# hszhao/semseg

Measured on NVIDIA H100. Metric: PSPNet50 473x473 training images/sec, higher is better.
Workload: dtype bf16

## Files before the change

semseg_b200/csrc/conv_igemm.cu:

```cuda
#include "host_common.h"
#include "ptx.cuh"

namespace sb {

constexpr int kBlockM = 128;
constexpr int kBlockK = 64;
constexpr int kConvThreads = 384;
constexpr int kConsumerThreads = 256;
constexpr int kATileBytes = kBlockM * kBlockK * 2;
constexpr int kStageOutBytes = kBlockM * 64 * 2;
constexpr int kMiscBytes = 2048;

template <int BLOCK_N>
struct ConvCfg {
  static constexpr int kBTileBytes = BLOCK_N * kBlockK * 2;
  static constexpr int kStageBytes = kATileBytes + kBTileBytes;
  static constexpr int kStages = (BLOCK_N == 256) ? 4 : (BLOCK_N == 128 ? 6 : 8);
  static constexpr int kSmemBytes = kStages * kStageBytes + 2 * kStageOutBytes + kMiscBytes + 1024;
};

struct ConvKParams {
  int N, H, W;
  int Cin, Cout;
  int taps;
  int bh, bw, tiles_h, tiles_w;
  int n_tiles, num_m_tiles;
  int k_chunks;
  int dh[SEMSEG_MAX_TAPS], dw[SEMSEG_MAX_TAPS], wtap[SEMSEG_MAX_TAPS], img_add[SEMSEG_MAX_TAPS];
  int img_mul;
  int epi_mode, relu;
  const float* scale;
  const float* shift;
  const __nv_bfloat16* residual;
  const __nv_bfloat16* residual_lo;
  int res_pitch;
  int nseg;
  int k_slices, kb_per_slice;
  long long slice_stride;
  float* out_f32;
  int out_pitch;
  float* stats_partial;
};

template <int BLOCK_N, bool kSplit>
__global__ void __launch_bounds__(kConvThreads, 1)
conv_igemm_kernel(const __grid_constant__ CUtensorMap tmA, const __grid_constant__ CUtensorMap tmB,
                  const __grid_constant__ CUtensorMap tmC, const __grid_constant__ CUtensorMap tmA_lo,
                  const __grid_constant__ CUtensorMap tmB_lo, const __grid_constant__ CUtensorMap tmC_lo,
                  const ConvKParams p) {
  using Cfg = ConvCfg<BLOCK_N>;
  constexpr int kStages = Cfg::kStages;
  constexpr int kStageBytes = Cfg::kStageBytes;
  constexpr int kAcc = BLOCK_N / 2;
  const int num_items = p.num_m_tiles * p.n_tiles * p.k_slices;
  auto decode_item = [&](int item, int& m_tile, int& n_tile, int& k_slice) {
    k_slice = item % p.k_slices;
    item /= p.k_slices;
    n_tile = item % p.n_tiles;
    m_tile = item / p.n_tiles;
  };

  extern __shared__ __align__(1024) uint8_t smem_raw[];
  uint8_t* smem = reinterpret_cast<uint8_t*>((reinterpret_cast<uintptr_t>(smem_raw) + 1023) & ~uintptr_t(1023));
  uint8_t* stage_base = smem;
  uint8_t* out_stage = smem + kStages * kStageBytes;
  uint8_t* misc = out_stage + 2 * kStageOutBytes;
  static_assert(kStages <= 16, "barrier area sized for <= 16 stages");
  uint64_t* full_bar = reinterpret_cast<uint64_t*>(misc);
  uint64_t* empty_bar = full_bar + 16;

  const int warp = threadIdx.x >> 5;
  const int lane = threadIdx.x & 31;
  const int nseg = kSplit ? p.nseg : 1;
  const int total_kblk = p.taps * p.k_chunks;
  auto slice_range = [&](int k_slice, int& kblk0, int& kblk1) {
    kblk0 = k_slice * p.kb_per_slice;
    kblk1 = min(kblk0 + p.kb_per_slice, total_kblk);
  };
  const uint32_t stage_tx = static_cast<uint32_t>(p.bh * p.bw) * 128u + static_cast<uint32_t>(Cfg::kBTileBytes);

  if (warp == 0 && lane == 0) {
    tma_prefetch_desc(&tmA);
    tma_prefetch_desc(&tmB);
    tma_prefetch_desc(&tmC);
    if (kSplit) {
      tma_prefetch_desc(&tmA_lo);
      tma_prefetch_desc(&tmB_lo);
      tma_prefetch_desc(&tmC_lo);
    }
    for (int i = 0; i < kStages; ++i) {
      mbar_init(&full_bar[i], 1);
      mbar_init(&empty_bar[i], kConsumerThreads);
    }
    fence_barrier_init();
  }
  if (p.stats_partial != nullptr) {
    float* row = p.stats_partial + static_cast<size_t>(blockIdx.x) * 4 * 3 * p.Cout;
    for (int i = threadIdx.x; i < 4 * 3 * p.Cout; i += kConvThreads) row[i] = 0.f;
  }
  __syncthreads();

  if (warp < 4) {
    setmaxnreg_dec<40>();
    if (warp == 0 && elect_one()) {
      int it = 0;
      for (int item = blockIdx.x; item < num_items; item += gridDim.x) {
        int m_tile, n_tile, k_slice, kblk0, kblk1;
        decode_item(item, m_tile, n_tile, k_slice);
        slice_range(k_slice, kblk0, kblk1);
        const int tiles_per_img = p.tiles_h * p.tiles_w;
        const int img = m_tile / tiles_per_img;
        const int rem = m_tile - img * tiles_per_img;
        const int h0 = (rem / p.tiles_w) * p.bh;
        const int w0 = (rem % p.tiles_w) * p.bw;
        const int n0 = n_tile * BLOCK_N;
        for (int kb = kblk0 * nseg; kb < kblk1 * nseg; ++kb, ++it) {
          const int s = it % kStages;
          const uint32_t par = (it / kStages) & 1;
          mbar_wait(&empty_bar[s], par ^ 1);
          const int ks = kb / nseg;
          const int seg = kb - ks * nseg;
          const int cb = ks / p.taps;
          const int t = ks - cb * p.taps;
          const CUtensorMap* mA = (kSplit && seg == 1) ? &tmA_lo : &tmA;
          const CUtensorMap* mB = (kSplit && seg == 2) ? &tmB_lo : &tmB;
          uint8_t* a_dst = stage_base + s * kStageBytes;
          uint8_t* b_dst = a_dst + kATileBytes;
          mbar_expect_tx(&full_bar[s], stage_tx);
          tma_load_4d(a_dst, mA, &full_bar[s], cb * kBlockK, w0 + p.dw[t], h0 + p.dh[t],
                      img * p.img_mul + p.img_add[t]);
          tma_load_3d(b_dst, mB, &full_bar[s], cb * kBlockK, n0, p.wtap[t]);
        }
      }
    }
  } else {
    setmaxnreg_inc<232>();
    const int ct = threadIdx.x - 128;
    const int wg = ct >> 7;
    const int wq = (ct >> 5) & 3;
    const int r_base = wg * 64 + wq * 16 + (lane >> 2);
    const int cq = 2 * (lane & 3);
    int it = 0;
    int store_buf = 0;
    float acc[kAcc];
    for (int item = blockIdx.x; item < num_items; item += gridDim.x) {
      int m_tile, n_tile, k_slice, kblk0, kblk1;
      decode_item(item, m_tile, n_tile, k_slice);
      slice_range(k_slice, kblk0, kblk1);
      const int num_kb = (kblk1 - kblk0) * nseg;
      int prev_s = -1;
#pragma unroll
      for (int i = 0; i < kAcc; ++i) acc[i] = 0.f;
      for (int kb = 0; kb < num_kb; ++kb, ++it) {
        const int s = it % kStages;
        const uint32_t par = (it / kStages) & 1;
        mbar_wait(&full_bar[s], par);
        const uint32_t a_addr = smem_u32(stage_base + s * kStageBytes) + static_cast<uint32_t>(wg * 64 * 128);
        const uint32_t b_addr = smem_u32(stage_base + s * kStageBytes + kATileBytes);
        const uint64_t adesc = make_wgmma_desc_sw128(a_addr, 16, 1024);
        const uint64_t bdesc = make_wgmma_desc_sw128(b_addr, 16, 1024);
        wgmma_fence_operand(acc);
        wgmma_fence();
#pragma unroll
        for (int k = 0; k < kBlockK / 16; ++k)
          wgmma_bf16<BLOCK_N, 0, 0>(acc, adesc + static_cast<uint64_t>(k * 2), bdesc + static_cast<uint64_t>(k * 2),
                                    (kb > 0 || k > 0) ? 1u : 0u);
        wgmma_commit();
        wgmma_wait<1>();
        wgmma_fence_operand(acc);
        if (prev_s >= 0) mbar_arrive(&empty_bar[prev_s]);
        prev_s = s;
      }
      wgmma_wait<0>();
      wgmma_fence_operand(acc);
      if (prev_s >= 0) mbar_arrive(&empty_bar[prev_s]);

      const int tiles_per_img = p.tiles_h * p.tiles_w;
      const int img = m_tile / tiles_per_img;
      const int rem = m_tile - img * tiles_per_img;
      const int h0 = (rem / p.tiles_w) * p.bh;
      const int w0 = (rem % p.tiles_w) * p.bw;
      const int n0 = n_tile * BLOCK_N;
      auto row_ok = [&](int r) {
        const int hi = r / p.bw, wi = r - (r / p.bw) * p.bw;
        return (r < p.bh * p.bw) && (h0 + hi < p.H) && (w0 + wi < p.W);
      };
      auto row_pix = [&](int r) {
        const int hi = r / p.bw, wi = r - hi * p.bw;
        return (static_cast<long long>(img) * p.H + (h0 + hi)) * p.W + (w0 + wi);
      };
      bool rv[2];
      long long pix[2];
#pragma unroll
      for (int i = 0; i < 2; ++i) {
        rv[i] = row_ok(r_base + 8 * i);
        pix[i] = row_pix(r_base + 8 * i);
      }
      constexpr int kChunks = BLOCK_N / 64;
#pragma unroll
      for (int ch = 0; ch < kChunks; ++ch) {
        const int c0 = n0 + ch * 64;
        if (c0 >= p.Cout) break;
        float* a = acc + ch * 32;

        if (p.epi_mode == SEMSEG_EPI_F32) {
          const bool bias = p.shift != nullptr && k_slice == 0;
          const bool pairs = (p.out_pitch & 1) == 0;
#pragma unroll
          for (int i = 0; i < 2; ++i) {
            if (!rv[i]) continue;
            float* orow = p.out_f32 + k_slice * p.slice_stride + pix[i] * p.out_pitch;
#pragma unroll
            for (int j = 0; j < 8; ++j) {
              const int c = c0 + 8 * j + cq;
              float v0 = a[4 * j + 2 * i], v1 = a[4 * j + 2 * i + 1];
              if (pairs && c + 1 < p.Cout) {
                if (bias) {
                  v0 += __ldg(p.shift + c);
                  v1 += __ldg(p.shift + c + 1);
                }
                *reinterpret_cast<float2*>(orow + c) = make_float2(v0, v1);
              } else {
                if (c < p.Cout) orow[c] = bias ? v0 + __ldg(p.shift + c) : v0;
                if (c + 1 < p.Cout) orow[c + 1] = bias ? v1 + __ldg(p.shift + c + 1) : v1;
              }
            }
          }
          continue;
        }

        if (p.epi_mode == SEMSEG_EPI_AFFINE) {
          const bool has_res = p.residual != nullptr;
#pragma unroll
          for (int j = 0; j < 8; ++j) {
            const int c = c0 + 8 * j + cq;
            const float sc0 = p.scale ? __ldg(p.scale + c) : 1.f, sc1 = p.scale ? __ldg(p.scale + c + 1) : 1.f;
            const float sh0 = p.shift ? __ldg(p.shift + c) : 0.f, sh1 = p.shift ? __ldg(p.shift + c + 1) : 0.f;
#pragma unroll
            for (int i = 0; i < 2; ++i) {
              float r0 = 0.f, r1 = 0.f;
              if (has_res && rv[i]) {
                const long long ro = pix[i] * p.res_pitch + c;
                float2 f = __bfloat1622float2(*reinterpret_cast<const __nv_bfloat162*>(p.residual + ro));
                if constexpr (kSplit) {
                  const float2 fl = __bfloat1622float2(*reinterpret_cast<const __nv_bfloat162*>(p.residual_lo + ro));
                  f.x += fl.x;
                  f.y += fl.y;
                }
                r0 = f.x;
                r1 = f.y;
              }
              float v0 = fmaf(a[4 * j + 2 * i], sc0, sh0) + r0;
              float v1 = fmaf(a[4 * j + 2 * i + 1], sc1, sh1) + r1;
              if (p.relu) {
                v0 = fmaxf(v0, 0.f);
                v1 = fmaxf(v1, 0.f);
              }
              a[4 * j + 2 * i] = v0;
              a[4 * j + 2 * i + 1] = v1;
            }
          }
        }

        uint8_t* obuf = out_stage + (kSplit ? 0 : store_buf) * kStageOutBytes;
        if (ct == 0) tma_store_wait_read<(kSplit ? 0 : 1)>();
        named_bar_sync(1, kConsumerThreads);
#pragma unroll
        for (int j = 0; j < 8; ++j) {
#pragma unroll
          for (int i = 0; i < 2; ++i) {
            const int r = r_base + 8 * i;
            const float v0 = a[4 * j + 2 * i], v1 = a[4 * j + 2 * i + 1];
            const uint32_t h = pack_bf16x2(v0, v1);
            const int off = r * 128 + ((j ^ (r & 7)) << 4) + cq * 2;
            *reinterpret_cast<uint32_t*>(obuf + off) = h;
            if constexpr (kSplit) {
              const float2 hf = __bfloat1622float2(*reinterpret_cast<const __nv_bfloat162*>(&h));
              *reinterpret_cast<uint32_t*>(obuf + kStageOutBytes + off) = pack_bf16x2(v0 - hf.x, v1 - hf.y);
            }
          }
        }
        fence_proxy_async_smem();
        named_bar_sync(1, kConsumerThreads);
        if (ct == 0) {
          tma_store_4d(&tmC, obuf, c0, w0, h0, img);
          if (kSplit) tma_store_4d(&tmC_lo, obuf + kStageOutBytes, c0, w0, h0, img);
          tma_store_commit();
        }
        if (p.stats_partial != nullptr && p.epi_mode == SEMSEG_EPI_RAW && wg == (ch & 1)) {
          const int g = wq;
          float* st_dst = p.stats_partial + (static_cast<size_t>(blockIdx.x) * 4 + g) * 3 * p.Cout + c0 + 2 * lane;
          float st_old[6];
          st_old[0] = st_dst[0];
          st_old[1] = st_dst[1];
          st_old[2] = st_dst[p.Cout];
          st_old[3] = st_dst[p.Cout + 1];
          st_old[4] = st_dst[2 * p.Cout];
          st_old[5] = st_dst[2 * p.Cout + 1];
          const uint32_t row_msk = __ballot_sync(0xffffffffu, row_ok(g * 32 + lane));
          float s0 = 0.f, s1 = 0.f, q0 = 0.f, q1 = 0.f;
          const uint8_t* base = obuf + (lane & 3) * 4;
          const int chunk16 = lane >> 2;
          auto add_row = [&](int rr, int sw) {
            float2 f = __bfloat1622float2(
                *reinterpret_cast<const __nv_bfloat162*>(base + rr * 128 + ((chunk16 ^ sw) << 4)));
            if constexpr (kSplit) {
              const float2 fl = __bfloat1622float2(*reinterpret_cast<const __nv_bfloat162*>(
                  base + kStageOutBytes + rr * 128 + ((chunk16 ^ sw) << 4)));
              f.x += fl.x;
              f.y += fl.y;
            }
            s0 += f.x;
            s1 += f.y;
            q0 = fmaf(f.x, f.x, q0);
            q1 = fmaf(f.y, f.y, q1);
          };
          if ((row_msk & (row_msk + 1u)) == 0u) {
            const int nr = __popc(row_msk);
            const int nfull = nr >> 3;
            for (int b8 = 0; b8 < nfull; ++b8) {
              const int rr0 = g * 32 + b8 * 8;
#pragma unroll
              for (int k = 0; k < 8; ++k) add_row(rr0 + k, k);
            }
            for (int r = nfull * 8; r < nr; ++r) add_row(g * 32 + r, r & 7);
          } else {
#pragma unroll
            for (int r = 0; r < 32; ++r)
              if ((row_msk >> r) & 1u) add_row(g * 32 + r, r & 7);
          }
          const float nt = static_cast<float>(__popc(row_msk));
          st_dst[0] = st_old[0] + s0;
          st_dst[1] = st_old[1] + s1;
          st_dst[p.Cout] = st_old[2] + q0;
          st_dst[p.Cout + 1] = st_old[3] + q1;
          st_dst[2 * p.Cout] = st_old[4] + nt;
          st_dst[2 * p.Cout + 1] = st_old[5] + nt;
        }
        store_buf ^= 1;
      }
    }
    if (ct == 0) tma_store_wait_all<0>();
  }
}

static int conv_grid(int num_m_tiles, int n_tiles) {
  const int sms = num_sms();
  const long long tiles = static_cast<long long>(num_m_tiles) * n_tiles;
  return static_cast<int>(tiles < sms ? tiles : sms);
}

struct ConvMaps {
  CUtensorMap a, b, c, a_lo, b_lo, c_lo;
};

template <int BLOCK_N>
static int launch_conv(const ConvMaps& tm, const ConvKParams& kp, bool split, int grid, cudaStream_t stream) {
  using Cfg = ConvCfg<BLOCK_N>;
  static std::atomic<bool> attr_set[64];
  int dev = 0;
  SB_CUDA(cudaGetDevice(&dev));
  if (dev < 0 || dev >= 64 || !attr_set[dev].load(std::memory_order_acquire)) {
    SB_CUDA(cudaFuncSetAttribute(conv_igemm_kernel<BLOCK_N, false>, cudaFuncAttributeMaxDynamicSharedMemorySize,
                                 Cfg::kSmemBytes));
    SB_CUDA(cudaFuncSetAttribute(conv_igemm_kernel<BLOCK_N, true>, cudaFuncAttributeMaxDynamicSharedMemorySize,
                                 Cfg::kSmemBytes));
    if (dev >= 0 && dev < 64) attr_set[dev].store(true, std::memory_order_release);
  }
  if (split)
    conv_igemm_kernel<BLOCK_N, true><<<grid, kConvThreads, Cfg::kSmemBytes, stream>>>(tm.a, tm.b, tm.c, tm.a_lo,
                                                                                      tm.b_lo, tm.c_lo, kp);
  else
    conv_igemm_kernel<BLOCK_N, false><<<grid, kConvThreads, Cfg::kSmemBytes, stream>>>(tm.a, tm.b, tm.c, tm.a_lo,
                                                                                       tm.b_lo, tm.c_lo, kp);
  SB_LAUNCHED();
  return SEMSEG_OK;
}

}

static int conv_block_n(int Cout) {
  if (Cout % 256 == 0 || Cout > 128) return 256;
  return Cout > 64 ? 128 : 64;
}

extern "C" int semseg_conv_k_slices(int Cin, int taps, int max_kblocks) {
  if (Cin <= 0 || taps <= 0 || max_kblocks <= 0) return SEMSEG_E_INVALID;
  const int total = taps * sb::cdiv(Cin, sb::kBlockK);
  const int per = sb::cdiv(total, sb::cdiv(total, max_kblocks));
  return sb::cdiv(total, per);
}

extern "C" int semseg_conv_stats_rows(int N, int H, int W, int Cout) {
  if (N <= 0 || H <= 0 || W <= 0 || Cout <= 0) return SEMSEG_E_INVALID;
  int bh, bw;
  sb::choose_box(H, W, sb::kBlockM, &bh, &bw);
  return 4 * sb::conv_grid(N * sb::cdiv(H, bh) * sb::cdiv(W, bw), sb::cdiv(Cout, conv_block_n(Cout)));
}

extern "C" int semseg_conv_fprop(const semseg_conv_desc* d, void* stream_) {
  using namespace sb;
  cudaStream_t stream = static_cast<cudaStream_t>(stream_);
  SB_CHECK_ARG(d != nullptr, "conv: null descriptor");
  SB_CHECK_ARG(d->N > 0 && d->H > 0 && d->W > 0 && d->Cin > 0 && d->Cout > 0, "conv: bad sizes");
  SB_CHECK_ARG(d->taps >= 1 && d->taps <= SEMSEG_MAX_TAPS, "conv: taps=%d out of range", d->taps);
  SB_CHECK_ARG(d->x && d->w, "conv: null x/w");
  SB_CHECK_ARG(d->x_pitch % 8 == 0 && d->x_pitch >= d->Cin, "conv: x_pitch %d must be a multiple of 8 and >= Cin",
               d->x_pitch);
  SB_CHECK_ARG(d->w_cols % 8 == 0 && d->w_cols >= d->Cin, "conv: w_cols %d must be a multiple of 8 and >= Cin",
               d->w_cols);
  SB_CHECK_ARG(d->epi_mode >= 0 && d->epi_mode <= 2, "conv: bad epi_mode");

  ConvKParams kp;
  memset(&kp, 0, sizeof(kp));
  kp.N = d->N; kp.H = d->H; kp.W = d->W; kp.Cin = d->Cin; kp.Cout = d->Cout; kp.taps = d->taps;
  choose_box(d->H, d->W, kBlockM, &kp.bh, &kp.bw);
  kp.tiles_h = cdiv(d->H, kp.bh);
  kp.tiles_w = cdiv(d->W, kp.bw);
  kp.num_m_tiles = d->N * kp.tiles_h * kp.tiles_w;
  kp.k_chunks = cdiv(d->Cin, kBlockK);
  for (int t = 0; t < d->taps; ++t) {
    kp.dh[t] = d->dh[t]; kp.dw[t] = d->dw[t]; kp.wtap[t] = d->wtap[t]; kp.img_add[t] = d->img_add[t];
    SB_CHECK_ARG(d->wtap[t] >= 0 && d->wtap[t] < d->n_wtaps, "conv: wtap[%d]=%d out of range", t, d->wtap[t]);
  }
  kp.img_mul = d->img_mul;
  kp.epi_mode = d->epi_mode; kp.relu = d->relu;
  kp.scale = d->scale; kp.shift = d->shift;
  kp.residual = static_cast<const __nv_bfloat16*>(d->residual); kp.res_pitch = d->res_pitch;
  kp.residual_lo = static_cast<const __nv_bfloat16*>(d->residual_lo);
  const bool split = d->x_lo != nullptr;
  kp.nseg = split ? 3 : 1;
  if (split) {
    SB_CHECK_ARG(d->w_split != 0, "conv: split activations need split weights (w_split)");
    SB_CHECK_ARG(d->epi_mode == SEMSEG_EPI_F32 || d->y_lo != nullptr, "conv: split input needs a split output (y_lo)");
    SB_CHECK_ARG(!d->residual || d->residual_lo, "conv: split input needs a split residual (residual_lo)");
  } else {
    SB_CHECK_ARG(!d->y_lo && !d->residual_lo, "conv: lo planes given without x_lo");
  }
  kp.out_f32 = d->out_f32; kp.out_pitch = d->out_pitch;
  kp.stats_partial = d->stats_partial;

  const int block_n = conv_block_n(d->Cout);
  kp.n_tiles = cdiv(d->Cout, block_n);
  kp.k_slices = 1;
  kp.kb_per_slice = kp.taps * kp.k_chunks;
  kp.slice_stride = 0;
  if (d->k_slices > 1) {
    SB_CHECK_ARG(d->epi_mode == SEMSEG_EPI_F32, "conv: K slicing needs the F32 epilogue (partials are fp32)");
    SB_CHECK_ARG(d->slice_stride >= static_cast<long long>(d->N) * d->H * d->W * d->out_pitch,
                 "conv: slice_stride too small for an [N,H,W,out_pitch] partial");
    kp.kb_per_slice = cdiv(kp.taps * kp.k_chunks, d->k_slices);
    kp.k_slices = cdiv(kp.taps * kp.k_chunks, kp.kb_per_slice);
    SB_CHECK_ARG(kp.k_slices == d->k_slices, "conv: k_slices %d not realisable for %d K blocks (use %d)", d->k_slices,
                 kp.taps * kp.k_chunks, kp.k_slices);
    kp.slice_stride = d->slice_stride;
  }
  const int grid = conv_grid(kp.num_m_tiles, kp.n_tiles * kp.k_slices);

  ConvMaps tm;
  {
    uint64_t dims[4] = {(uint64_t)d->Cin, (uint64_t)d->Win, (uint64_t)d->Hin, (uint64_t)d->Nin};
    uint64_t str[3] = {(uint64_t)d->x_pitch * 2, (uint64_t)d->x_pitch * 2 * d->Win,
                       (uint64_t)d->x_pitch * 2 * d->Win * d->Hin};
    uint32_t box[4] = {(uint32_t)kBlockK, (uint32_t)kp.bw, (uint32_t)kp.bh, 1};
    int r = encode_tmap_bf16(&tm.a, d->x, 4, dims, str, box);
    if (r) return r;
    tm.a_lo = tm.a;
    if (split && (r = encode_tmap_bf16(&tm.a_lo, d->x_lo, 4, dims, str, box))) return r;
  }
  {
    uint64_t dims[3] = {(uint64_t)d->w_cols, (uint64_t)d->w_rows, (uint64_t)d->n_wtaps};
    uint64_t str[2] = {(uint64_t)d->w_cols * 2, (uint64_t)d->w_cols * 2 * d->w_rows};
    uint32_t box[3] = {(uint32_t)kBlockK, (uint32_t)block_n, 1};
    int r = encode_tmap_bf16(&tm.b, d->w, 3, dims, str, box);
    if (r) return r;
    tm.b_lo = tm.b;
    if (split) {
      const __nv_bfloat16* w_lo =
          static_cast<const __nv_bfloat16*>(d->w) + static_cast<size_t>(d->n_wtaps) * d->w_rows * d->w_cols;
      if ((r = encode_tmap_bf16(&tm.b_lo, w_lo, 3, dims, str, box))) return r;
    }
  }
  if (d->epi_mode == SEMSEG_EPI_F32) {
    SB_CHECK_ARG(d->out_f32 != nullptr && d->out_pitch >= d->Cout, "conv: F32 epilogue needs out_f32/out_pitch");
    tm.c = tm.a;
    tm.c_lo = tm.a;
  } else {
    SB_CHECK_ARG(d->y != nullptr, "conv: null y");
    SB_CHECK_ARG(d->Cout % 64 == 0, "conv: bf16 epilogue needs Cout %% 64 == 0 (got %d)", d->Cout);
    SB_CHECK_ARG(d->y_pitch % 8 == 0 && d->y_pitch >= d->Cout, "conv: bad y_pitch %d", d->y_pitch);
    if (d->residual) SB_CHECK_ARG(d->res_pitch % 8 == 0, "conv: res_pitch must be a multiple of 8");
    uint64_t dims[4] = {(uint64_t)d->Cout, (uint64_t)d->W, (uint64_t)d->H, (uint64_t)d->N};
    uint64_t str[3] = {(uint64_t)d->y_pitch * 2, (uint64_t)d->y_pitch * 2 * d->W,
                       (uint64_t)d->y_pitch * 2 * d->W * d->H};
    uint32_t box[4] = {64u, (uint32_t)kp.bw, (uint32_t)kp.bh, 1};
    int r = encode_tmap_bf16(&tm.c, d->y, 4, dims, str, box);
    if (r) return r;
    tm.c_lo = tm.c;
    if (split && (r = encode_tmap_bf16(&tm.c_lo, d->y_lo, 4, dims, str, box))) return r;
  }
  switch (block_n) {
    case 256: return launch_conv<256>(tm, kp, split, grid, stream);
    case 128: return launch_conv<128>(tm, kp, split, grid, stream);
    default: return launch_conv<64>(tm, kp, split, grid, stream);
  }
}
```

semseg_b200/csrc/host_common.cu:

```cuda
#include "host_common.h"

#include <cudaTypedefs.h>
#include <stdarg.h>
#include <string.h>

#include <mutex>

namespace sb {

static thread_local char g_err[512] = "";
std::atomic<long long> g_launches{0};

void set_error(const char* fmt, ...) {
  va_list ap;
  va_start(ap, fmt);
  vsnprintf(g_err, sizeof(g_err), fmt, ap);
  va_end(ap);
}

int num_sms() {
  static int cached[64] = {0};
  int dev = 0;
  if (cudaGetDevice(&dev) != cudaSuccess || dev < 0 || dev >= 64) return 148;
  if (cached[dev] == 0) {
// ... 2 lines not shown
    cached[dev] = n;
  }
  return cached[dev];
}

static PFN_cuTensorMapEncodeTiled_v12000 get_encode() {
  static PFN_cuTensorMapEncodeTiled_v12000 fn = nullptr;
  static std::once_flag once;
  std::call_once(once, [] {
    void* p = nullptr;
    cudaDriverEntryPointQueryResult q;
    if (cudaGetDriverEntryPoint("cuTensorMapEncodeTiled", &p, cudaEnableDefault, &q) == cudaSuccess &&
        q == cudaDriverEntryPointSuccess)
      fn = reinterpret_cast<PFN_cuTensorMapEncodeTiled_v12000>(p);
  });
  return fn;
}

int encode_tmap_bf16(CUtensorMap* out, const void* base, int rank, const uint64_t* dims,
                     const uint64_t* strides_bytes, const uint32_t* box) {
  auto fn = get_encode();
  if (!fn) {
    set_error("cuTensorMapEncodeTiled entry point unavailable (no CUDA driver?)");
    return SEMSEG_E_CUDA;
  }
  if ((reinterpret_cast<uintptr_t>(base) & 15) != 0) {
    set_error("tensor base %p not 16-byte aligned", base);
    return SEMSEG_E_INVALID;
  }
  cuuint64_t gd[5];
  cuuint64_t gs[4];
  cuuint32_t bx[5], es[5];
  for (int i = 0; i < rank; ++i) {
    gd[i] = dims[i];
    bx[i] = box[i];
    es[i] = 1;
    if (box[i] == 0 || box[i] > 256) {
      set_error("TMA box dim %d = %u out of range", i, box[i]);
      return SEMSEG_E_INVALID;
    }
  }
  for (int i = 0; i + 1 < rank; ++i) {
    gs[i] = strides_bytes[i];
    if (gs[i] % 16 != 0) {
      set_error("TMA stride %d = %llu not a multiple of 16 bytes", i, (unsigned long long)gs[i]);
      return SEMSEG_E_INVALID;
    }
  }
  CUresult r = fn(out, CU_TENSOR_MAP_DATA_TYPE_BFLOAT16, rank, const_cast<void*>(base), gd, gs, bx, es,
                  CU_TENSOR_MAP_INTERLEAVE_NONE, CU_TENSOR_MAP_SWIZZLE_128B, CU_TENSOR_MAP_L2_PROMOTION_L2_256B,
                  CU_TENSOR_MAP_FLOAT_OOB_FILL_NONE);
  if (r != CUDA_SUCCESS) {
    set_error("cuTensorMapEncodeTiled failed with CUresult %d (rank %d dims %llu,%llu,%llu box %u,%u,%u)", (int)r,
              rank, (unsigned long long)gd[0], (unsigned long long)gd[1], (unsigned long long)(rank > 2 ? gd[2] : 0),
              bx[0], bx[1], rank > 2 ? bx[2] : 0);
    return SEMSEG_E_CUDA;
  }
  return SEMSEG_OK;
}

void choose_box(int H, int W, int max_pixels, int* bh_out, int* bw_out) {
  double best = -1.0;
  int best_bh = 1, best_bw = 1;
  int wcap = W < max_pixels ? W : max_pixels;
  for (int bw = 1; bw <= wcap; ++bw) {
    int bh = max_pixels / bw;
    if (bh > H) bh = H;
    if (bh > 256) bh = 256;
    if (bh < 1) continue;
    int th = cdiv(H, bh);
    bh = cdiv(H, th);
    int tw = cdiv(W, bw);
    double util = (double)H * W / ((double)th * tw * max_pixels);
    if (util > best + 1e-9 || (util > best - 1e-9 && bw > best_bw)) {
      best = util;
      best_bh = bh;
      best_bw = bw;
    }
  }
  *bh_out = best_bh;
  *bw_out = best_bw;
}

}

extern "C" const char* semseg_last_error(void) { return sb::g_err; }
extern "C" int semseg_abi_version(void) { return 1; }
extern "C" long long semseg_launch_count(void) { return sb::g_launches.load(); }
```

semseg_b200/csrc/host_common.h:

```cpp
#pragma once
#include <cuda.h>
#include <cuda_runtime.h>
#include <stdint.h>
#include <stdio.h>

#include <atomic>

#include "../../include/semseg_b200.h"

namespace sb {

void set_error(const char* fmt, ...);
extern std::atomic<long long> g_launches;
int num_sms();

#define SB_CHECK_ARG(cond, ...)  \
  do {                           \
    if (!(cond)) {               \
      sb::set_error(__VA_ARGS__); \
      return SEMSEG_E_INVALID;   \
    }                            \
  } while (0)

#define SB_CUDA(call)                                                                     \
  do {                                                                                    \
    cudaError_t e__ = (call);                                                             \
    if (e__ != cudaSuccess) {                                                             \
      sb::set_error("%s failed: %s (%s:%d)", #call, cudaGetErrorString(e__), __FILE__, __LINE__); \
      return SEMSEG_E_CUDA;                                                               \
    }                                                                                     \
  } while (0)

#define SB_LAUNCHED()                                                                        \
  do {                                                                                       \
    sb::g_launches.fetch_add(1, std::memory_order_relaxed);                                  \
    cudaError_t e__ = cudaGetLastError();                                                    \
    if (e__ != cudaSuccess) {                                                                \
      sb::set_error("kernel launch failed: %s (%s:%d)", cudaGetErrorString(e__), __FILE__, __LINE__); \
      return SEMSEG_E_CUDA;                                                                  \
    }                                                                                        \
  } while (0)

int encode_tmap_bf16(CUtensorMap* out, const void* base, int rank, const uint64_t* dims,
                     const uint64_t* strides_bytes, const uint32_t* box);

void choose_box(int H, int W, int max_pixels, int* bh, int* bw);

static inline int cdiv(int a, int b) { return (a + b - 1) / b; }

}
```

semseg_b200/csrc/ptx.cuh:

```cuda
#pragma once
#include <cuda.h>
#include <cuda_runtime.h>
#include <cuda_bf16.h>
#include <stdint.h>

namespace sb {

__device__ __forceinline__ uint32_t smem_u32(const void* p) {
  return static_cast<uint32_t>(__cvta_generic_to_shared(p));
}

__device__ __forceinline__ bool elect_one() {
  uint32_t pred = 0;
  asm volatile(
      "{\n"
      ".reg .pred P1;\n"
      "elect.sync _|P1, 0xffffffff;\n"
      "selp.u32 %0, 1, 0, P1;\n"
      "}\n"
      : "=r"(pred));
  return pred != 0;
}

__device__ __forceinline__ void mbar_init(uint64_t* bar, uint32_t count) {
  asm volatile("mbarrier.init.shared::cta.b64 [%0], %1;" ::"r"(smem_u32(bar)), "r"(count));
}
__device__ __forceinline__ void fence_barrier_init() {
  asm volatile("fence.mbarrier_init.release.cluster;" ::: "memory");
}
__device__ __forceinline__ void mbar_expect_tx(uint64_t* bar, uint32_t bytes) {
  asm volatile("mbarrier.arrive.expect_tx.shared::cta.b64 _, [%0], %1;" ::"r"(smem_u32(bar)), "r"(bytes)
               : "memory");
}
__device__ __forceinline__ void mbar_arrive(uint64_t* bar) {
  asm volatile("mbarrier.arrive.shared::cta.b64 _, [%0];" ::"r"(smem_u32(bar)) : "memory");
}
__device__ __forceinline__ bool mbar_try_wait(uint64_t* bar, uint32_t parity) {
  uint32_t ok;
  asm volatile(
      "{\n"
      ".reg .pred P1;\n"
      "mbarrier.try_wait.parity.shared::cta.b64 P1, [%1], %2;\n"
      "selp.u32 %0, 1, 0, P1;\n"
      "}\n"
      : "=r"(ok)
      : "r"(smem_u32(bar)), "r"(parity)
      : "memory");
  return ok != 0;
}
__device__ __forceinline__ void mbar_wait(uint64_t* bar, uint32_t parity) {
  if (mbar_try_wait(bar, parity)) return;
  long long t0 = clock64();
  while (!mbar_try_wait(bar, parity)) {
    if (clock64() - t0 > 8000000000LL) __trap();
  }
}

__device__ __forceinline__ void fence_proxy_async_smem() {
  asm volatile("fence.proxy.async.shared::cta;" ::: "memory");
}
__device__ __forceinline__ void named_bar_sync(uint32_t id, uint32_t nthreads) {
  asm volatile("bar.sync %0, %1;" ::"r"(id), "r"(nthreads) : "memory");
}

__device__ __forceinline__ void tma_prefetch_desc(const CUtensorMap* m) {
  asm volatile("prefetch.tensormap [%0];" ::"l"(reinterpret_cast<uint64_t>(m)) : "memory");
}
__device__ __forceinline__ void tma_load_2d(void* dst, const CUtensorMap* m, uint64_t* bar, int c0, int c1) {
  asm volatile(
      "cp.async.bulk.tensor.2d.shared::cluster.global.mbarrier::complete_tx::bytes [%0], [%1, {%3, %4}], [%2];"
      ::"r"(smem_u32(dst)), "l"(reinterpret_cast<uint64_t>(m)), "r"(smem_u32(bar)), "r"(c0), "r"(c1)
      : "memory");
}
__device__ __forceinline__ void tma_load_3d(void* dst, const CUtensorMap* m, uint64_t* bar, int c0, int c1, int c2) {
  asm volatile(
      "cp.async.bulk.tensor.3d.shared::cluster.global.mbarrier::complete_tx::bytes [%0], [%1, {%3, %4, %5}], [%2];"
      ::"r"(smem_u32(dst)), "l"(reinterpret_cast<uint64_t>(m)), "r"(smem_u32(bar)), "r"(c0), "r"(c1), "r"(c2)
      : "memory");
}
__device__ __forceinline__ void tma_load_4d(void* dst, const CUtensorMap* m, uint64_t* bar, int c0, int c1, int c2,
                                            int c3) {
  asm volatile(
      "cp.async.bulk.tensor.4d.shared::cluster.global.mbarrier::complete_tx::bytes [%0], [%1, {%3, %4, %5, %6}], "
      "[%2];" ::"r"(smem_u32(dst)),
      "l"(reinterpret_cast<uint64_t>(m)), "r"(smem_u32(bar)), "r"(c0), "r"(c1), "r"(c2), "r"(c3)
      : "memory");
}
__device__ __forceinline__ void tma_store_4d(const CUtensorMap* m, const void* src, int c0, int c1, int c2, int c3) {
  asm volatile("cp.async.bulk.tensor.4d.global.shared::cta.bulk_group [%0, {%2, %3, %4, %5}], [%1];" ::"l"(
                   reinterpret_cast<uint64_t>(m)),
               "r"(smem_u32(src)), "r"(c0), "r"(c1), "r"(c2), "r"(c3)
               : "memory");
}
__device__ __forceinline__ void tma_store_commit() { asm volatile("cp.async.bulk.commit_group;" ::: "memory"); }
template <int N>
__device__ __forceinline__ void tma_store_wait_read() {
  asm volatile("cp.async.bulk.wait_group.read %0;" ::"n"(N) : "memory");
}
template <int N>
__device__ __forceinline__ void tma_store_wait_all() {
  asm volatile("cp.async.bulk.wait_group %0;" ::"n"(N) : "memory");
}

template <int R>
__device__ __forceinline__ void setmaxnreg_dec() {
  asm volatile("setmaxnreg.dec.sync.aligned.u32 %0;" ::"n"(R));
}
template <int R>
__device__ __forceinline__ void setmaxnreg_inc() {
  asm volatile("setmaxnreg.inc.sync.aligned.u32 %0;" ::"n"(R));
}

__device__ __forceinline__ void wgmma_fence() { asm volatile("wgmma.fence.sync.aligned;" ::: "memory"); }
__device__ __forceinline__ void wgmma_commit() { asm volatile("wgmma.commit_group.sync.aligned;" ::: "memory"); }
template <int N>
__device__ __forceinline__ void wgmma_wait() {
  asm volatile("wgmma.wait_group.sync.aligned %0;" ::"n"(N) : "memory");
}
template <int R>
__device__ __forceinline__ void wgmma_fence_operand(float (&d)[R]) {
#pragma unroll
  for (int i = 0; i < R; ++i) asm volatile("" : "+f"(d[i])::"memory");
}

__device__ __forceinline__ uint64_t make_wgmma_desc_sw128(uint32_t smem_addr, uint32_t lbo_bytes, uint32_t sbo_bytes) {
  uint64_t d = 0;
  d |= static_cast<uint64_t>((smem_addr & 0x3FFFF) >> 4);
  d |= static_cast<uint64_t>((lbo_bytes >> 4) & 0x3FFF) << 16;
  d |= static_cast<uint64_t>((sbo_bytes >> 4) & 0x3FFF) << 32;
  d |= static_cast<uint64_t>(1) << 62;
  return d;
}

template <int TA, int TB>
__device__ __forceinline__ void wgmma_m64n64(float (&d)[32], uint64_t adesc, uint64_t bdesc, uint32_t accumulate) {
  asm volatile(
      "{\n"
      ".reg .pred p;\n"
      "setp.ne.b32 p, %34, 0;\n"
      "wgmma.mma_async.sync.aligned.m64n64k16.f32.bf16.bf16 "
      "{%0, %1, %2, %3, %4, %5, %6, %7, %8, %9, %10, %11, %12, %13, %14, %15, %16, %17, %18, %19, %20, %21, %22, %23, %24, %25, %26, %27, %28, %29, %30, %31}, "
      "%32, %33, p, 1, 1, %35, %36;\n"
      "}\n"
      : "+f"(d[0]), "+f"(d[1]), "+f"(d[2]), "+f"(d[3]), "+f"(d[4]), "+f"(d[5]), "+f"(d[6]), "+f"(d[7]), "+f"(d[8]), "+f"(d[9]), "+f"(d[10]), "+f"(d[11]), "+f"(d[12]), "+f"(d[13]), "+f"(d[14]), "+f"(d[15]), "+f"(d[16]), "+f"(d[17]), "+f"(d[18]), "+f"(d[19]), "+f"(d[20]), "+f"(d[21]), "+f"(d[22]), "+f"(d[23]), "+f"(d[24]), "+f"(d[25]), "+f"(d[26]), "+f"(d[27]), "+f"(d[28]), "+f"(d[29]), "+f"(d[30]), "+f"(d[31])
      : "l"(adesc), "l"(bdesc), "r"(accumulate), "n"(TA), "n"(TB));
}

template <int TA, int TB>
__device__ __forceinline__ void wgmma_m64n128(float (&d)[64], uint64_t adesc, uint64_t bdesc, uint32_t accumulate) {
  asm volatile(
      "{\n"
      ".reg .pred p;\n"
      "setp.ne.b32 p, %66, 0;\n"
      "wgmma.mma_async.sync.aligned.m64n128k16.f32.bf16.bf16 "
      "{%0, %1, %2, %3, %4, %5, %6, %7, %8, %9, %10, %11, %12, %13, %14, %15, %16, %17, %18, %19, %20, %21, %22, %23, %24, %25, %26, %27, %28, %29, %30, %31, %32, %33, %34, %35, %36, %37, %38, %39, %40, %41, %42, %43, %44, %45, %46, %47, %48, %49, %50, %51, %52, %53, %54, %55, %56, %57, %58, %59, %60, %61, %62, %63}, "
      "%64, %65, p, 1, 1, %67, %68;\n"
      "}\n"
      : "+f"(d[0]), "+f"(d[1]), "+f"(d[2]), "+f"(d[3]), "+f"(d[4]), "+f"(d[5]), "+f"(d[6]), "+f"(d[7]), "+f"(d[8]), "+f"(d[9]), "+f"(d[10]), "+f"(d[11]), "+f"(d[12]), "+f"(d[13]), "+f"(d[14]), "+f"(d[15]), "+f"(d[16]), "+f"(d[17]), "+f"(d[18]), "+f"(d[19]), "+f"(d[20]), "+f"(d[21]), "+f"(d[22]), "+f"(d[23]), "+f"(d[24]), "+f"(d[25]), "+f"(d[26]), "+f"(d[27]), "+f"(d[28]), "+f"(d[29]), "+f"(d[30]), "+f"(d[31]), "+f"(d[32]), "+f"(d[33]), "+f"(d[34]), "+f"(d[35]), "+f"(d[36]), "+f"(d[37]), "+f"(d[38]), "+f"(d[39]), "+f"(d[40]), "+f"(d[41]), "+f"(d[42]), "+f"(d[43]), "+f"(d[44]), "+f"(d[45]), "+f"(d[46]), "+f"(d[47]), "+f"(d[48]), "+f"(d[49]), "+f"(d[50]), "+f"(d[51]), "+f"(d[52]), "+f"(d[53]), "+f"(d[54]), "+f"(d[55]), "+f"(d[56]), "+f"(d[57]), "+f"(d[58]), "+f"(d[59]), "+f"(d[60]), "+f"(d[61]), "+f"(d[62]), "+f"(d[63])
      : "l"(adesc), "l"(bdesc), "r"(accumulate), "n"(TA), "n"(TB));
}

template <int TA, int TB>
__device__ __forceinline__ void wgmma_m64n256(float (&d)[128], uint64_t adesc, uint64_t bdesc, uint32_t accumulate) {
  asm volatile(
      "{\n"
      ".reg .pred p;\n"
      "setp.ne.b32 p, %130, 0;\n"
      "wgmma.mma_async.sync.aligned.m64n256k16.f32.bf16.bf16 "
      "{%0, %1, %2, %3, %4, %5, %6, %7, %8, %9, %10, %11, %12, %13, %14, %15, %16, %17, %18, %19, %20, %21, %22, %23, %24, %25, %26, %27, %28, %29, %30, %31, %32, %33, %34, %35, %36, %37, %38, %39, %40, %41, %42, %43, %44, %45, %46, %47, %48, %49, %50, %51, %52, %53, %54, %55, %56, %57, %58, %59, %60, %61, %62, %63, %64, %65, %66, %67, %68, %69, %70, %71, %72, %73, %74, %75, %76, %77, %78, %79, %80, %81, %82, %83, %84, %85, %86, %87, %88, %89, %90, %91, %92, %93, %94, %95, %96, %97, %98, %99, %100, %101, %102, %103, %104, %105, %106, %107, %108, %109, %110, %111, %112, %113, %114, %115, %116, %117, %118, %119, %120, %121, %122, %123, %124, %125, %126, %127}, "
// ... 21 lines not shown
```

Baseline: 285.6.

## Use TMA im2col loads with flat 128-pixel M tiles for non-stats convolutions

```diff
diff --git a/semseg_b200/csrc/conv_igemm.cu b/semseg_b200/csrc/conv_igemm.cu
--- a/semseg_b200/csrc/conv_igemm.cu
+++ b/semseg_b200/csrc/conv_igemm.cu
@@ -20,13 +20,16 @@
 };
 
 struct ConvKParams {
-  int N, H, W;
+  int H, W;
+  int M;
   int Cin, Cout;
   int taps;
-  int bh, bw, tiles_h, tiles_w;
   int n_tiles, num_m_tiles;
   int k_chunks;
-  int dh[SEMSEG_MAX_TAPS], dw[SEMSEG_MAX_TAPS], wtap[SEMSEG_MAX_TAPS], img_add[SEMSEG_MAX_TAPS];
+  int lo_w, lo_h;
+  int wtap[SEMSEG_MAX_TAPS], amap[SEMSEG_MAX_TAPS], off_w[SEMSEG_MAX_TAPS], off_h[SEMSEG_MAX_TAPS];
+  int boxes, bh, bw, tiles_h, tiles_w;
+  int dh[SEMSEG_MAX_TAPS], dw[SEMSEG_MAX_TAPS], img_add[SEMSEG_MAX_TAPS];
   int img_mul;
   int epi_mode, relu;
   const float* scale;
@@ -42,12 +45,14 @@
   float* stats_partial;
 };
 
+struct ConvMaps {
+  CUtensorMap a[kMaxInputMaps], a_lo[kMaxInputMaps];
+  CUtensorMap b, b_lo, c, c_lo;
+};
+
 template <int BLOCK_N, bool kSplit>
 __global__ void __launch_bounds__(kConvThreads, 1)
-conv_igemm_kernel(const __grid_constant__ CUtensorMap tmA, const __grid_constant__ CUtensorMap tmB,
-                  const __grid_constant__ CUtensorMap tmC, const __grid_constant__ CUtensorMap tmA_lo,
-                  const __grid_constant__ CUtensorMap tmB_lo, const __grid_constant__ CUtensorMap tmC_lo,
-                  const ConvKParams p) {
+conv_igemm_kernel(const __grid_constant__ ConvMaps tm, const ConvKParams p) {
   using Cfg = ConvCfg<BLOCK_N>;
   constexpr int kStages = Cfg::kStages;
   constexpr int kStageBytes = Cfg::kStageBytes;
@@ -77,16 +82,18 @@
     kblk0 = k_slice * p.kb_per_slice;
     kblk1 = min(kblk0 + p.kb_per_slice, total_kblk);
   };
-  const uint32_t stage_tx = static_cast<uint32_t>(p.bh * p.bw) * 128u + static_cast<uint32_t>(Cfg::kBTileBytes);
+  const uint32_t a_bytes = p.boxes ? static_cast<uint32_t>(p.bh * p.bw) * 128u : static_cast<uint32_t>(kATileBytes);
+  const uint32_t stage_tx = a_bytes + static_cast<uint32_t>(Cfg::kBTileBytes);
+  const int HW = p.H * p.W;
 
   if (warp == 0 && lane == 0) {
-    tma_prefetch_desc(&tmA);
-    tma_prefetch_desc(&tmB);
-    tma_prefetch_desc(&tmC);
+    tma_prefetch_desc(&tm.a[0]);
+    tma_prefetch_desc(&tm.b);
+    tma_prefetch_desc(&tm.c);
     if (kSplit) {
-      tma_prefetch_desc(&tmA_lo);
-      tma_prefetch_desc(&tmB_lo);
-      tma_prefetch_desc(&tmC_lo);
+      tma_prefetch_desc(&tm.a_lo[0]);
+      tma_prefetch_desc(&tm.b_lo);
+      tma_prefetch_desc(&tm.c_lo);
     }
     for (int i = 0; i < kStages; ++i) {
       mbar_init(&full_bar[i], 1);
@@ -108,11 +115,20 @@
         int m_tile, n_tile, k_slice, kblk0, kblk1;
         decode_item(item, m_tile, n_tile, k_slice);
         slice_range(k_slice, kblk0, kblk1);
-        const int tiles_per_img = p.tiles_h * p.tiles_w;
-        const int img = m_tile / tiles_per_img;
-        const int rem = m_tile - img * tiles_per_img;
-        const int h0 = (rem / p.tiles_w) * p.bh;
-        const int w0 = (rem % p.tiles_w) * p.bw;
+        int img, h0, w0;
+        if (p.boxes) {
+          const int tiles_per_img = p.tiles_h * p.tiles_w;
+          img = m_tile / tiles_per_img;
+          const int rem = m_tile - img * tiles_per_img;
+          h0 = (rem / p.tiles_w) * p.bh;
+          w0 = (rem % p.tiles_w) * p.bw;
+        } else {
+          const int m0 = m_tile * kBlockM;
+          img = m0 / HW;
+          const int rem = m0 - img * HW;
+          h0 = rem / p.W + p.lo_h;
+          w0 = rem - (rem / p.W) * p.W + p.lo_w;
+        }
         const int n0 = n_tile * BLOCK_N;
         for (int kb = kblk0 * nseg; kb < kblk1 * nseg; ++kb, ++it) {
           const int s = it % kStages;
@@ -122,13 +138,17 @@
           const int seg = kb - ks * nseg;
           const int cb = ks / p.taps;
           const int t = ks - cb * p.taps;
-          const CUtensorMap* mA = (kSplit && seg == 1) ? &tmA_lo : &tmA;
-          const CUtensorMap* mB = (kSplit && seg == 2) ? &tmB_lo : &tmB;
+          const CUtensorMap* mA = (kSplit && seg == 1) ? &tm.a_lo[p.amap[t]] : &tm.a[p.amap[t]];
+          const CUtensorMap* mB = (kSplit && seg == 2) ? &tm.b_lo : &tm.b;
           uint8_t* a_dst = stage_base + s * kStageBytes;
           uint8_t* b_dst = a_dst + kATileBytes;
           mbar_expect_tx(&full_bar[s], stage_tx);
-          tma_load_4d(a_dst, mA, &full_bar[s], cb * kBlockK, w0 + p.dw[t], h0 + p.dh[t],
-                      img * p.img_mul + p.img_add[t]);
+          if (p.boxes)
+            tma_load_4d(a_dst, mA, &full_bar[s], cb * kBlockK, w0 + p.dw[t], h0 + p.dh[t],
+                        img * p.img_mul + p.img_add[t]);
+          else
+            tma_load_im2col_4d(a_dst, mA, &full_bar[s], cb * kBlockK, w0, h0, img,
+                               static_cast<uint16_t>(p.off_w[t]), static_cast<uint16_t>(p.off_h[t]));
           tma_load_3d(b_dst, mB, &full_bar[s], cb * kBlockK, n0, p.wtap[t]);
         }
       }
@@ -175,17 +195,24 @@
       wgmma_fence_operand(acc);
       if (prev_s >= 0) mbar_arrive(&empty_bar[prev_s]);
 
-      const int tiles_per_img = p.tiles_h * p.tiles_w;
-      const int img = m_tile / tiles_per_img;
-      const int rem = m_tile - img * tiles_per_img;
-      const int h0 = (rem / p.tiles_w) * p.bh;
-      const int w0 = (rem % p.tiles_w) * p.bw;
+      const int m0 = m_tile * kBlockM;
+      const int rows = min(kBlockM, p.M - m0);
+      int img = 0, h0 = 0, w0 = 0;
+      if (p.boxes) {
+        const int tiles_per_img = p.tiles_h * p.tiles_w;
+        img = m_tile / tiles_per_img;
+        const int rem = m_tile - img * tiles_per_img;
+        h0 = (rem / p.tiles_w) * p.bh;
+        w0 = (rem % p.tiles_w) * p.bw;
+      }
       const int n0 = n_tile * BLOCK_N;
       auto row_ok = [&](int r) {
+        if (!p.boxes) return r < rows;
         const int hi = r / p.bw, wi = r - (r / p.bw) * p.bw;
         return (r < p.bh * p.bw) && (h0 + hi < p.H) && (w0 + wi < p.W);
       };
       auto row_pix = [&](int r) {
+        if (!p.boxes) return static_cast<long long>(m0) + r;
         const int hi = r / p.bw, wi = r - hi * p.bw;
         return (static_cast<long long>(img) * p.H + (h0 + hi)) * p.W + (w0 + wi);
       };
@@ -283,8 +310,13 @@
         fence_proxy_async_smem();
         named_bar_sync(1, kConsumerThreads);
         if (ct == 0) {
-          tma_store_4d(&tmC, obuf, c0, w0, h0, img);
-          if (kSplit) tma_store_4d(&tmC_lo, obuf + kStageOutBytes, c0, w0, h0, img);
+          if (p.boxes) {
+            tma_store_4d(&tm.c, obuf, c0, w0, h0, img);
+            if (kSplit) tma_store_4d(&tm.c_lo, obuf + kStageOutBytes, c0, w0, h0, img);
+          } else {
+            tma_store_2d(&tm.c, obuf, c0, m0);
+            if (kSplit) tma_store_2d(&tm.c_lo, obuf + kStageOutBytes, c0, m0);
+          }
           tma_store_commit();
         }
         if (p.stats_partial != nullptr && p.epi_mode == SEMSEG_EPI_RAW && wg == (ch & 1)) {
@@ -350,10 +382,6 @@
   return static_cast<int>(tiles < sms ? tiles : sms);
 }
 
-struct ConvMaps {
-  CUtensorMap a, b, c, a_lo, b_lo, c_lo;
-};
-
 template <int BLOCK_N>
 static int launch_conv(const ConvMaps& tm, const ConvKParams& kp, bool split, int grid, cudaStream_t stream) {
   using Cfg = ConvCfg<BLOCK_N>;
@@ -368,11 +396,9 @@
     if (dev >= 0 && dev < 64) attr_set[dev].store(true, std::memory_order_release);
   }
   if (split)
-    conv_igemm_kernel<BLOCK_N, true><<<grid, kConvThreads, Cfg::kSmemBytes, stream>>>(tm.a, tm.b, tm.c, tm.a_lo,
-                                                                                      tm.b_lo, tm.c_lo, kp);
+    conv_igemm_kernel<BLOCK_N, true><<<grid, kConvThreads, Cfg::kSmemBytes, stream>>>(tm, kp);
   else
-    conv_igemm_kernel<BLOCK_N, false><<<grid, kConvThreads, Cfg::kSmemBytes, stream>>>(tm.a, tm.b, tm.c, tm.a_lo,
-                                                                                       tm.b_lo, tm.c_lo, kp);
+    conv_igemm_kernel<BLOCK_N, false><<<grid, kConvThreads, Cfg::kSmemBytes, stream>>>(tm, kp);
   SB_LAUNCHED();
   return SEMSEG_OK;
 }
@@ -391,6 +417,11 @@
   return sb::cdiv(total, per);
 }
 
+static long long conv_pixels(int N, int H, int W) {
+  const long long m = static_cast<long long>(N) * H * W;
+  return m <= 0x7fffffffLL - sb::kBlockM ? m : -1;
+}
+
 extern "C" int semseg_conv_stats_rows(int N, int H, int W, int Cout) {
   if (N <= 0 || H <= 0 || W <= 0 || Cout <= 0) return SEMSEG_E_INVALID;
   int bh, bw;
@@ -403,6 +434,9 @@
   cudaStream_t stream = static_cast<cudaStream_t>(stream_);
   SB_CHECK_ARG(d != nullptr, "conv: null descriptor");
   SB_CHECK_ARG(d->N > 0 && d->H > 0 && d->W > 0 && d->Cin > 0 && d->Cout > 0, "conv: bad sizes");
+  SB_CHECK_ARG(d->Nin > 0 && d->Hin > 0 && d->Win > 0, "conv: bad input sizes");
+  SB_CHECK_ARG(conv_pixels(d->N, d->H, d->W) > 0, "conv: %d x %d x %d output pixels do not fit an int", d->N, d->H,
+               d->W);
   SB_CHECK_ARG(d->taps >= 1 && d->taps <= SEMSEG_MAX_TAPS, "conv: taps=%d out of range", d->taps);
   SB_CHECK_ARG(d->x && d->w, "conv: null x/w");
   SB_CHECK_ARG(d->x_pitch % 8 == 0 && d->x_pitch >= d->Cin, "conv: x_pitch %d must be a multiple of 8 and >= Cin",
@@ -413,14 +447,28 @@
 
   ConvKParams kp;
   memset(&kp, 0, sizeof(kp));
-  kp.N = d->N; kp.H = d->H; kp.W = d->W; kp.Cin = d->Cin; kp.Cout = d->Cout; kp.taps = d->taps;
-  choose_box(d->H, d->W, kBlockM, &kp.bh, &kp.bw);
-  kp.tiles_h = cdiv(d->H, kp.bh);
-  kp.tiles_w = cdiv(d->W, kp.bw);
-  kp.num_m_tiles = d->N * kp.tiles_h * kp.tiles_w;
+  kp.H = d->H; kp.W = d->W; kp.Cin = d->Cin; kp.Cout = d->Cout; kp.taps = d->taps;
+  kp.M = d->N * d->H * d->W;
+  kp.boxes = d->stats_partial != nullptr;
+  if (kp.boxes) {
+    choose_box(d->H, d->W, kBlockM, &kp.bh, &kp.bw);
+    kp.tiles_h = cdiv(d->H, kp.bh);
+    kp.tiles_w = cdiv(d->W, kp.bw);
+    kp.num_m_tiles = d->N * kp.tiles_h * kp.tiles_w;
+  } else {
+    kp.num_m_tiles = cdiv(kp.M, kBlockM);
+  }
   kp.k_chunks = cdiv(d->Cin, kBlockK);
+  Im2colPlan plan;
+  {
+    const int r = plan_im2col(d->H, d->W, d->Nin, d->Hin, d->Win, d->taps, d->dh, d->dw, d->img_mul, d->img_add,
+                              &plan);
+    if (r) return r;
+  }
+  kp.lo_w = plan.lo_w; kp.lo_h = plan.lo_h;
   for (int t = 0; t < d->taps; ++t) {
-    kp.dh[t] = d->dh[t]; kp.dw[t] = d->dw[t]; kp.wtap[t] = d->wtap[t]; kp.img_add[t] = d->img_add[t];
+    kp.wtap[t] = d->wtap[t]; kp.amap[t] = kp.boxes ? 0 : plan.map[t]; kp.off_w[t] = plan.off_w[t]; kp.off_h[t] = plan.off_h[t];
+    kp.dh[t] = d->dh[t]; kp.dw[t] = d->dw[t]; kp.img_add[t] = d->img_add[t];
     SB_CHECK_ARG(d->wtap[t] >= 0 && d->wtap[t] < d->n_wtaps, "conv: wtap[%d]=%d out of range", t, d->wtap[t]);
   }
   kp.img_mul = d->img_mul;
@@ -457,16 +505,32 @@
   }
   const int grid = conv_grid(kp.num_m_tiles, kp.n_tiles * kp.k_slices);
 
+  if (d->epi_mode == SEMSEG_EPI_F32) {
+    SB_CHECK_ARG(d->out_f32 != nullptr && d->out_pitch >= d->Cout, "conv: F32 epilogue needs out_f32/out_pitch");
+  } else {
+    SB_CHECK_ARG(d->y != nullptr, "conv: null y");
+    SB_CHECK_ARG(d->Cout % 64 == 0, "conv: bf16 epilogue needs Cout %% 64 == 0 (got %d)", d->Cout);
+    SB_CHECK_ARG(d->y_pitch % 8 == 0 && d->y_pitch >= d->Cout, "conv: bad y_pitch %d", d->y_pitch);
+    if (d->residual) SB_CHECK_ARG(d->res_pitch % 8 == 0, "conv: res_pitch must be a multiple of 8");
+  }
+
   ConvMaps tm;
-  {
+  memset(&tm, 0, sizeof(tm));
+  if (kp.boxes) {
     uint64_t dims[4] = {(uint64_t)d->Cin, (uint64_t)d->Win, (uint64_t)d->Hin, (uint64_t)d->Nin};
     uint64_t str[3] = {(uint64_t)d->x_pitch * 2, (uint64_t)d->x_pitch * 2 * d->Win,
                        (uint64_t)d->x_pitch * 2 * d->Win * d->Hin};
     uint32_t box[4] = {(uint32_t)kBlockK, (uint32_t)kp.bw, (uint32_t)kp.bh, 1};
-    int r = encode_tmap_bf16(&tm.a, d->x, 4, dims, str, box);
+    int r = encode_tmap_bf16(&tm.a[0], d->x, 4, dims, str, box);
     if (r) return r;
-    tm.a_lo = tm.a;
-    if (split && (r = encode_tmap_bf16(&tm.a_lo, d->x_lo, 4, dims, str, box))) return r;
+    if (split && (r = encode_tmap_bf16(&tm.a_lo[0], d->x_lo, 4, dims, str, box))) return r;
+  } else {
+    int r = encode_im2col_maps(tm.a, d->x, d->Cin, d->x_pitch, d->N, d->Nin, d->Hin, d->Win, d->img_mul, plan, kBlockM);
+    if (r) return r;
+    if (split &&
+        (r = encode_im2col_maps(tm.a_lo, d->x_lo, d->Cin, d->x_pitch, d->N, d->Nin, d->Hin, d->Win, d->img_mul,
+                                plan, kBlockM)))
+      return r;
   }
   {
     uint64_t dims[3] = {(uint64_t)d->w_cols, (uint64_t)d->w_rows, (uint64_t)d->n_wtaps};
@@ -481,23 +545,21 @@
       if ((r = encode_tmap_bf16(&tm.b_lo, w_lo, 3, dims, str, box))) return r;
     }
   }
-  if (d->epi_mode == SEMSEG_EPI_F32) {
-    SB_CHECK_ARG(d->out_f32 != nullptr && d->out_pitch >= d->Cout, "conv: F32 epilogue needs out_f32/out_pitch");
-    tm.c = tm.a;
-    tm.c_lo = tm.a;
-  } else {
-    SB_CHECK_ARG(d->y != nullptr, "conv: null y");
-    SB_CHECK_ARG(d->Cout % 64 == 0, "conv: bf16 epilogue needs Cout %% 64 == 0 (got %d)", d->Cout);
-    SB_CHECK_ARG(d->y_pitch % 8 == 0 && d->y_pitch >= d->Cout, "conv: bad y_pitch %d", d->y_pitch);
-    if (d->residual) SB_CHECK_ARG(d->res_pitch % 8 == 0, "conv: res_pitch must be a multiple of 8");
+  if (d->epi_mode != SEMSEG_EPI_F32 && kp.boxes) {
     uint64_t dims[4] = {(uint64_t)d->Cout, (uint64_t)d->W, (uint64_t)d->H, (uint64_t)d->N};
     uint64_t str[3] = {(uint64_t)d->y_pitch * 2, (uint64_t)d->y_pitch * 2 * d->W,
                        (uint64_t)d->y_pitch * 2 * d->W * d->H};
     uint32_t box[4] = {64u, (uint32_t)kp.bw, (uint32_t)kp.bh, 1};
     int r = encode_tmap_bf16(&tm.c, d->y, 4, dims, str, box);
     if (r) return r;
-    tm.c_lo = tm.c;
     if (split && (r = encode_tmap_bf16(&tm.c_lo, d->y_lo, 4, dims, str, box))) return r;
+  } else if (d->epi_mode != SEMSEG_EPI_F32) {
+    uint64_t dims[2] = {(uint64_t)d->Cout, (uint64_t)kp.M};
+    uint64_t str[1] = {(uint64_t)d->y_pitch * 2};
+    uint32_t box[2] = {64u, (uint32_t)kBlockM};
+    int r = encode_tmap_bf16(&tm.c, d->y, 2, dims, str, box);
+    if (r) return r;
+    if (split && (r = encode_tmap_bf16(&tm.c_lo, d->y_lo, 2, dims, str, box))) return r;
   }
   switch (block_n) {
     case 256: return launch_conv<256>(tm, kp, split, grid, stream);
diff --git a/semseg_b200/csrc/host_common.cu b/semseg_b200/csrc/host_common.cu
--- a/semseg_b200/csrc/host_common.cu
+++ b/semseg_b200/csrc/host_common.cu
@@ -108,6 +108,86 @@
   *bw_out = best_bw;
 }
 
+static PFN_cuTensorMapEncodeIm2col_v12000 get_encode_im2col() {
+  static PFN_cuTensorMapEncodeIm2col_v12000 fn = nullptr;
+  static std::once_flag once;
+  std::call_once(once, [] {
+    void* p = nullptr;
+    cudaDriverEntryPointQueryResult q;
+    if (cudaGetDriverEntryPoint("cuTensorMapEncodeIm2col", &p, cudaEnableDefault, &q) == cudaSuccess &&
+        q == cudaDriverEntryPointSuccess)
+      fn = reinterpret_cast<PFN_cuTensorMapEncodeIm2col_v12000>(p);
+  });
+  return fn;
+}
+
+int plan_im2col(int H, int W, int Nin, int Hin, int Win, int taps, const int* dh, const int* dw, int img_mul,
+                const int* img_add, Im2colPlan* plan) {
+  SB_CHECK_ARG(img_mul >= 1, "conv: img_mul %d must be >= 1", img_mul);
+  memset(plan, 0, sizeof(*plan));
+  int lo_w = dw[0], lo_h = dh[0];
+  for (int t = 1; t < taps; ++t) {
+    lo_w = dw[t] < lo_w ? dw[t] : lo_w;
+    lo_h = dh[t] < lo_h ? dh[t] : lo_h;
+  }
+  const long long up_w = static_cast<long long>(lo_w) + W - Win, up_h = static_cast<long long>(lo_h) + H - Hin;
+  SB_CHECK_ARG(lo_w >= -128 && lo_w <= 127 && lo_h >= -128 && lo_h <= 127 && up_w >= -128 && up_w <= 127 &&
+                   up_h >= -128 && up_h <= 127,
+               "conv: tap shifts / grid sizes need im2col corners in [-128, 127] (lower %d,%d upper %lld,%lld)", lo_w,
+               lo_h, up_w, up_h);
+  plan->lo_w = lo_w;
+  plan->lo_h = lo_h;
+  plan->up_w = static_cast<int>(up_w);
+  plan->up_h = static_cast<int>(up_h);
+  for (int t = 0; t < taps; ++t) {
+    const long long ow = static_cast<long long>(dw[t]) - lo_w, oh = static_cast<long long>(dh[t]) - lo_h;
+    SB_CHECK_ARG(ow <= 65535 && oh <= 65535, "conv: tap %d shift (%d,%d) too far from the others", t, dh[t], dw[t]);
+    plan->off_w[t] = static_cast<int>(ow);
+    plan->off_h[t] = static_cast<int>(oh);
+    SB_CHECK_ARG(img_add[t] >= 0 && img_add[t] < Nin, "conv: img_add[%d] = %d outside the %d input images", t,
+                 img_add[t], Nin);
+    int k = 0;
+    while (k < plan->n_maps && plan->img_add[k] != img_add[t]) ++k;
+    if (k == plan->n_maps) {
+      SB_CHECK_ARG(k < kMaxInputMaps, "conv: more than %d distinct img_add values", kMaxInputMaps);
+      plan->img_add[plan->n_maps++] = img_add[t];
+    }
+    plan->map[t] = k;
+  }
+  return SEMSEG_OK;
+}
+
+int encode_im2col_maps(CUtensorMap* maps, const void* x, int C, int pitch, int N, int Nin, int Hin, int Win,
+                       int img_mul, const Im2colPlan& plan, uint32_t pixels) {
+  auto fn = get_encode_im2col();
+  if (!fn) {
+    set_error("cuTensorMapEncodeIm2col entry point unavailable (no CUDA driver?)");
+    return SEMSEG_E_CUDA;
+  }
+  const uint64_t img_bytes = static_cast<uint64_t>(pitch) * 2 * Win * Hin;
+  for (int k = 0; k < plan.n_maps; ++k) {
+    const uint8_t* base = static_cast<const uint8_t*>(x) + img_bytes * plan.img_add[k];
+    if ((reinterpret_cast<uintptr_t>(base) & 15) != 0 || pitch % 8 != 0) {
+      set_error("im2col tensor base %p / pitch %d not 16-byte aligned", base, pitch);
+      return SEMSEG_E_INVALID;
+    }
+    const int images = cdiv(Nin - plan.img_add[k], img_mul);
+    cuuint64_t gd[4] = {(cuuint64_t)C, (cuuint64_t)Win, (cuuint64_t)Hin, (cuuint64_t)(images < N ? images : N)};
+    cuuint64_t gs[3] = {(cuuint64_t)pitch * 2, (cuuint64_t)pitch * 2 * Win, img_bytes * img_mul};
+    cuuint32_t es[4] = {1, 1, 1, 1};
+    const int lower[2] = {plan.lo_w, plan.lo_h}, upper[2] = {plan.up_w, plan.up_h};
+    CUresult r = fn(&maps[k], CU_TENSOR_MAP_DATA_TYPE_BFLOAT16, 4, const_cast<uint8_t*>(base), gd, gs, lower, upper,
+                    64, pixels, es, CU_TENSOR_MAP_INTERLEAVE_NONE, CU_TENSOR_MAP_SWIZZLE_128B,
+                    CU_TENSOR_MAP_L2_PROMOTION_L2_256B, CU_TENSOR_MAP_FLOAT_OOB_FILL_NONE);
+    if (r != CUDA_SUCCESS) {
+      set_error("cuTensorMapEncodeIm2col failed with CUresult %d (dims %d,%d,%d,%llu corners %d,%d / %d,%d)", (int)r,
+                C, Win, Hin, (unsigned long long)gd[3], plan.lo_w, plan.lo_h, plan.up_w, plan.up_h);
+      return SEMSEG_E_CUDA;
+    }
+  }
+  return SEMSEG_OK;
+}
+
 }
 
 extern "C" const char* semseg_last_error(void) { return sb::g_err; }
diff --git a/semseg_b200/csrc/host_common.h b/semseg_b200/csrc/host_common.h
--- a/semseg_b200/csrc/host_common.h
+++ b/semseg_b200/csrc/host_common.h
@@ -46,6 +46,19 @@
 
 void choose_box(int H, int W, int max_pixels, int* bh, int* bw);
 
+constexpr int kMaxInputMaps = 4;
+struct Im2colPlan {
+  int lo_w, lo_h, up_w, up_h;
+  int n_maps;
+  int img_add[kMaxInputMaps];
+  int map[SEMSEG_MAX_TAPS];
+  int off_w[SEMSEG_MAX_TAPS], off_h[SEMSEG_MAX_TAPS];
+};
+int plan_im2col(int H, int W, int Nin, int Hin, int Win, int taps, const int* dh, const int* dw, int img_mul,
+                const int* img_add, Im2colPlan* plan);
+int encode_im2col_maps(CUtensorMap* maps, const void* x, int C, int pitch, int N, int Nin, int Hin, int Win,
+                       int img_mul, const Im2colPlan& plan, uint32_t pixels);
+
 static inline int cdiv(int a, int b) { return (a + b - 1) / b; }
 
 }
diff --git a/semseg_b200/csrc/ptx.cuh b/semseg_b200/csrc/ptx.cuh
--- a/semseg_b200/csrc/ptx.cuh
+++ b/semseg_b200/csrc/ptx.cuh
@@ -85,6 +85,20 @@
       "[%2];" ::"r"(smem_u32(dst)),
       "l"(reinterpret_cast<uint64_t>(m)), "r"(smem_u32(bar)), "r"(c0), "r"(c1), "r"(c2), "r"(c3)
       : "memory");
+}
+__device__ __forceinline__ void tma_load_im2col_4d(void* dst, const CUtensorMap* m, uint64_t* bar, int c, int w, int h,
+                                                   int n, uint16_t off_w, uint16_t off_h) {
+  asm volatile(
+      "cp.async.bulk.tensor.4d.shared::cluster.global.im2col.mbarrier::complete_tx::bytes [%0], [%1, {%3, %4, %5, %6}], "
+      "[%2], {%7, %8};" ::"r"(smem_u32(dst)),
+      "l"(reinterpret_cast<uint64_t>(m)), "r"(smem_u32(bar)), "r"(c), "r"(w), "r"(h), "r"(n), "h"(off_w), "h"(off_h)
+      : "memory");
+}
+__device__ __forceinline__ void tma_store_2d(const CUtensorMap* m, const void* src, int c0, int c1) {
+  asm volatile("cp.async.bulk.tensor.2d.global.shared::cta.bulk_group [%0, {%2, %3}], [%1];" ::"l"(
+                   reinterpret_cast<uint64_t>(m)),
+               "r"(smem_u32(src)), "r"(c0), "r"(c1)
+               : "memory");
 }
 __device__ __forceinline__ void tma_store_4d(const CUtensorMap* m, const void* src, int c0, int c1, int c2, int c3) {
   asm volatile("cp.async.bulk.tensor.4d.global.shared::cta.bulk_group [%0, {%2, %3, %4, %5}], [%1];" ::"l"(
```

Result: no change. 288.5, median of 6 (+1.0%).
